# giltchcity/orb_slam3_ros

Measured on AMD Instinct MI355X. Metric: frames/sec ORB extract+match (752×480, 1000 kp) at 1/2/4/8 GPU; % HBM roofline, higher is better.
Workload: dtype u8; 1 GPU; EuRoC-MH01-like stereo 752x480 (BASELINE config 2): ORBextractor L+R (nFeatures=1000, scale 1.2, 8 levels, FAST 20/7) + ComputeStereoMatches; width=752, height=480, allgather=False, pipelines=1, parallelism=frame-sharded x1

## Files before the change

### include/orbfe.h

```cpp
#ifndef ORBFE_H
#define ORBFE_H

#include <stdint.h>

#ifdef __cplusplus
extern "C" {
#endif

#define ORBFE_OK 0
#define ORBFE_E_EMPTY (-1)
#define ORBFE_E_ARG (-2)
#define ORBFE_E_DEVICE (-3)
#define ORBFE_E_CAPACITY (-4)

typedef struct orbfe_keypoint {
    float x, y, size, angle, response;
    int32_t octave, class_id;
} orbfe_keypoint;

typedef struct orbfe_extractor orbfe_extractor;


int orbfe_extractor_create(int nfeatures, float scaleFactor, int nlevels, int iniThFAST, int minThFAST,
                           orbfe_extractor** out);
// ... 460 lines not shown
int orbfe_kfdb_detect_nbest(orbfe_kfdb* db, const uint32_t* q_word_ids, const double* q_weights, int32_t q_n,
                            const int32_t* connected_ids, int32_t n_connected, int32_t map_id,
                            const int32_t* bad_map_ids, int32_t n_bad_maps, int32_t n_candidates,
                            orbfe_kf_info_fn info, void* ctx, int32_t* loop_ids, int32_t* n_loop,
                            int32_t* merge_ids, int32_t* n_merge);

int orbfe_remap_linear_batch(const uint8_t* const* d_src, int sw, int sh, int sstride, const float* d_mapx,
                             const float* d_mapy, int dw, int dh, uint8_t* const* d_dst, int dstride, int n,
                             void* stream);
int orbfe_remap_linear(const uint8_t* src, int sw, int sh, int sstride, const float* mapx, const float* mapy, int dw,
                       int dh, uint8_t* dst, int dstride);

int orbfe_undistort_points(const float* pts, int n, const float* K4, const float* dist, int ndist, float* out);

int orbfe_matcher_set_timing(int enable);
float orbfe_matcher_last_ms(void);
int orbfe_matcher_set_stats(int enable);
int orbfe_matcher_last_stats(long long* out);
enum {
    ORBFE_SBP_FORM_NONE = 0,
    ORBFE_SBP_FORM_BLOCK = 1,
    ORBFE_SBP_FORM_MULTI = 2,
    ORBFE_SBP_FORM_BAND = 3,
    ORBFE_SBP_FORM_LOCAL = 4,
    ORBFE_SBP_FORM_LOCAL_WQ0 = 5,
    ORBFE_SBP_FORM_LOCAL_WQ1 = 6,
    ORBFE_SBP_FORM_LOCAL_WQ2 = 7,
    ORBFE_SBP_FORM_PROJ = 8,
    ORBFE_SBP_FORM_BLOCK4 = 9,
    ORBFE_SBP_FORM_BLOCK2 = 10,
    ORBFE_SBP_FORM_LOCAL2 = 11,
    ORBFE_SBP_FORM_PROJ2 = 12
};
int orbfe_matcher_last_form(void);
enum {
    ORBFE_BOW_FORM_NONE = 0,
    ORBFE_BOW_FORM_BLOCK = 1,
    ORBFE_BOW_FORM_NODES = 2,
    ORBFE_BOW_FORM_KFKF = 3
};
int orbfe_matcher_last_bow_form(void);
int orbfe_matcher_last_bow_batch(int32_t* out);
int orbfe_matcher_last_knn_form(int32_t* out);
int orbfe_matcher_last_bow_kf_batch(int32_t* out);
int orbfe_matcher_last_tri_batch(int32_t* out);
int orbfe_matcher_last_fuse_batch(int32_t* out);
int orbfe_matcher_last_track_batch(int32_t* out);
int orbfe_matcher_last_local_batch(int32_t* out);
int orbfe_matcher_last_local_uploads(void);
int orbfe_matcher_last_sim3_passes(void);

int orbfe_debug_copy(orbfe_extractor* h, int what, int image, int level, void* dst, int cap_bytes);

int orbfe_debug_fill_extractor(orbfe_extractor* h, uint32_t word, int64_t* bytes_out);

int orbfe_debug_fill_matcher(uint32_t word, int64_t bytes_out[3]);

int orbfe_debug_block_sort(uint64_t* data, int n);

const char* orbfe_version(void);

int orbfe_copy_stream(const void* d_src, void* d_dst, size_t bytes, void* stream);

#ifdef __cplusplus
}
#endif
#endif
```

### orb_slam3_ros_amd/_lib.py

```python
from __future__ import annotations

import ctypes
import os

_HERE = os.path.dirname(os.path.abspath(__file__))
LIB_PATH = os.path.join(_HERE, "liborbfe.so")
HEADER_PATH = os.path.join(os.path.dirname(_HERE), "include", "orbfe.h")

ORBFE_OK = 0
ORBFE_E_EMPTY = -1
ORBFE_E_ARG = -2
ORBFE_E_DEVICE = -3
ORBFE_E_CAPACITY = -4
ORBFE_NUM_STAGES = 3
STAGE_NAMES = ("pyramid_fast", "octree", "describe")


EPIPOLAR_FN = ctypes.CFUNCTYPE(ctypes.c_int32, ctypes.c_void_p, ctypes.c_int32, ctypes.c_int32)
KF_INFO_FN = ctypes.CFUNCTYPE(ctypes.c_int32, ctypes.c_void_p, ctypes.c_int32, ctypes.POINTER(ctypes.c_int32),
                              ctypes.POINTER(ctypes.c_int32))


class OrbKeyPoint(ctypes.Structure):
    _fields_ = [("x", ctypes.c_float), ("y", ctypes.c_float), ("size", ctypes.c_float),
                ("angle", ctypes.c_float), ("response", ctypes.c_float),
                ("octave", ctypes.c_int32), ("class_id", ctypes.c_int32)]


ORBFE_DEPTH_U16 = 0
ORBFE_DEPTH_F32 = 1


class RGBDParamsStruct(ctypes.Structure):
    _fields_ = [("fx", ctypes.c_float), ("fy", ctypes.c_float), ("cx", ctypes.c_float), ("cy", ctypes.c_float),
                ("dist", ctypes.c_float * 12), ("ndist", ctypes.c_int32), ("bf", ctypes.c_float),
                ("depth_factor", ctypes.c_float)]


class BowBatchStruct(ctypes.Structure):
    _fields_ = [("bow_word_ids", ctypes.c_void_p), ("bow_weights", ctypes.c_void_p), ("fv_node_ids", ctypes.c_void_p),
                ("fv_offsets", ctypes.c_void_p), ("fv_indices", ctypes.c_void_p), ("counts", ctypes.c_void_p)]


_c_int, _c_float, _vp = ctypes.c_int, ctypes.c_float, ctypes.c_void_p
_P_int, _P_float = ctypes.POINTER(ctypes.c_int), ctypes.POINTER(ctypes.c_float)

_SIGS = {
    "orbfe_extractor_create": (_c_int, [_c_int, _c_float, _c_int, _c_int, _c_int, ctypes.POINTER(_vp)]),
    "orbfe_extractor_destroy": (None, [_vp]),
    "orbfe_extractor_levels": (_c_int, [_vp]),
    "orbfe_extractor_scale_info": (_c_int, [_vp, _vp, _vp, _vp, _vp, _vp]),
    "orbfe_extractor_capacity": (_c_int, [_vp, _c_int, _c_int]),
    "orbfe_extract": (_c_int, [_vp, _vp, _c_int, _c_int, _c_int, _c_int, _c_int, _vp, _vp, _c_int, _P_int]),
    "orbfe_pyramid_level": (_c_int, [_vp, _c_int, _c_int, _vp, _c_int, _P_int, _P_int]),
    "orbfe_extract_batch": (_c_int, [_vp, _c_int, _vp, _c_int, _c_int, _c_int, _c_int, _c_int, _vp]),
    "orbfe_extract_batch_laps": (_c_int, [_vp, _c_int, _vp, _c_int, _c_int, _c_int, _vp, _vp]),
    "orbfe_batch_outputs": (_c_int, [_vp, ctypes.POINTER(_vp), ctypes.POINTER(_vp), ctypes.POINTER(_vp), _P_int]),
    "orbfe_set_stage_timing": (_c_int, [_vp, _c_int]),
    "orbfe_extractor_set_opencv_model": (_c_int, [_vp, _c_int, _c_int]),
    "orbfe_extractor_get_opencv_model": (_c_int, [_vp, _P_int, _P_int]),
    "orbfe_set_batch_outputs": (_c_int, [_vp, _vp, _vp, _vp, _c_int]),
    "orbfe_get_stage_timing": (_c_int, [_vp, _vp]),
    "orbfe_get_call_timing": (_c_int, [_vp, _vp]),
    "orbfe_stereo_match_batch": (_c_int, [_vp, _c_int, _c_int, _vp, _c_int, _c_int, _c_int, _c_float, _c_float,
                                          _vp, _vp, _vp, _vp]),
    "orbfe_stereo_match": (_c_int, [_vp, _vp, _c_float, _c_float, _vp, _vp]),
    "orbfe_frame_stereo": (_c_int, [_vp, _vp, _vp, _vp, _c_int, _c_int, _c_int, _c_float, _c_float,
                                    _vp, _vp, _c_int, _P_int, _P_int, _vp, _vp, _c_int, _P_int, _P_int, _vp, _vp]),
    "orbfe_frame_fisheye": (_c_int, [_vp, _vp, _vp, _vp, _c_int, _c_int, _c_int, _c_int, _c_int, _c_float,
                                     _vp, _vp, _c_int, _P_int, _P_int, _vp, _vp, _c_int, _P_int, _P_int, _vp, _vp]),
    "orbfe_descriptor_distance": (_c_int, [_vp, _vp]),
    "orbfe_debug_copy": (_c_int, [_vp, _c_int, _c_int, _c_int, _vp, _c_int]),
    "orbfe_debug_fill_extractor": (_c_int, [_vp, ctypes.c_uint32, ctypes.POINTER(ctypes.c_int64)]),
    "orbfe_debug_fill_matcher": (_c_int, [ctypes.c_uint32, ctypes.POINTER(ctypes.c_int64)]),
    "orbfe_debug_block_sort": (_c_int, [_vp, _c_int]),
    "orbfe_version": (ctypes.c_char_p, []),
    "orbfe_search_by_projection_local": (_c_int, [_vp, _vp, _vp, _vp, _c_int, _c_float, _c_int, _c_float, _c_float]),
    "orbfe_search_by_projection_lastframe": (_c_int, [_vp, _vp, _vp, _vp, _c_int, _c_float, _c_int, _c_int, _c_int]),
    "orbfe_search_by_projection_lastframe_stereo": (_c_int, [_vp, _vp, _vp, _vp, _vp, _c_int, _c_float, _c_int, _c_int,
                                                             _c_int]),
    "orbfe_search_by_projection_lastframe_pose": (_c_int, [_vp, _vp, _vp, _vp, _c_int, _vp, _vp, _vp, _c_float, _c_int,
                                                           _c_int, _c_int]),
    "orbfe_search_by_projection_kf": (_c_int, [_vp, _vp, _vp, _c_int, _c_float, _c_int, _c_int]),
    "orbfe_search_for_initialization": (_c_int, [_vp, _vp, _vp, _vp, _c_int, _c_float, _c_int]),
    "orbfe_search_by_bow": (_c_int, [_vp, _vp, _vp, _c_int, _vp, _vp, _vp, _vp, _c_float, _c_int]),
    "orbfe_copy_stream": (_c_int, [_vp, _vp, ctypes.c_size_t, _vp]),
    "orbfe_search_by_projection_local_device": (_c_int, [_vp, _vp, _vp, _vp, _c_int, _c_float, _c_int, _c_float,
                                                         _c_float, _vp]),
    "orbfe_search_local_points_device": (_c_int, [_vp, _vp, _vp, _c_int, _vp, _vp, _c_float, _c_int, _c_float,
                                                  _c_float, _vp, _vp]),
    "orbfe_search_by_bow_kf": (_c_int, [_vp, _vp, _vp, _c_int, _vp, _vp, _vp, _vp, _c_int, _vp, _vp, _c_float,
                                        _c_int]),
    "orbfe_distinctive_descriptors": (_c_int, [_vp, _vp, _c_int, _vp]),
    "orbfe_search_for_triangulation": (_c_int, [_vp, _vp, _vp, _vp, _vp, _vp, _vp, _vp, _vp, _c_int, _c_int, _c_int,
                                                _vp]),
    "orbfe_fuse": (_c_int, [_vp, _vp, _vp, _vp, _c_int, _c_float, _c_int, _vp, _vp]),
    "orbfe_search_by_projection_sim3": (_c_int, [_vp, _vp, _vp, _c_int, _vp, _c_int, _c_float, _vp, _vp]),
    "orbfe_search_by_projection_sim3_rig": (_c_int, [_vp, _vp, _vp, _vp, _c_int, _vp, _c_int, _c_float, _vp, _vp]),
    "orbfe_search_for_triangulation_epi": (_c_int, [_vp, _vp, _vp, _vp, _vp, _vp, _vp, _c_int, _c_int, EPIPOLAR_FN,
                                                    _vp, _vp]),
    "orbfe_search_by_sim3": (_c_int, [_vp, _vp, _vp, _vp, _vp, _vp, _vp, _vp, _c_float, _vp, _vp]),
    "orbfe_stereo_knn_ratio": (_c_int, [_vp, _c_int, _vp, _c_int, _c_float, _vp, _vp]),
    "orbfe_stereo_knn_slabs": (_c_int, [_vp, _vp, _c_int, _c_int, _vp, _vp, _c_int, _c_int, _c_int, _c_int, _c_float,
                                        _vp, _vp, _vp, _vp]),
    "orbfe_stereo_knn_batch": (_c_int, [_vp, _c_int, _c_int, _vp, _c_int, _c_int, _c_int, _c_float, _vp, _vp, _vp,
                                        _vp]),
    "orbfe_matcher_set_timing": (_c_int, [_c_int]),
    "orbfe_matcher_set_stats": (_c_int, [_c_int]),
    "orbfe_matcher_last_stats": (_c_int, [_vp]),
    "orbfe_matcher_last_form": (_c_int, []),
    "orbfe_matcher_last_bow_form": (_c_int, []),
    "orbfe_matcher_last_bow_batch": (_c_int, [_vp]),
    "orbfe_matcher_last_knn_form": (_c_int, [_vp]),
    "orbfe_matcher_last_sim3_passes": (_c_int, []),
    "orbfe_undistort_points": (_c_int, [_vp, _c_int, _vp, _vp, _c_int, _vp]),
    "orbfe_remap_linear": (_c_int, [_vp, _c_int, _c_int, _c_int, _vp, _vp, _c_int, _c_int, _vp, _c_int]),
    "orbfe_remap_linear_batch": (_c_int, [_vp, _c_int, _c_int, _c_int, _vp, _vp, _c_int, _c_int, _vp, _c_int, _c_int, _vp]),
    "orbfe_vocabulary_load_bin": (_c_int, [_vp, ctypes.c_size_t, ctypes.POINTER(_vp)]),
    "orbfe_vocabulary_create": (_c_int, [_c_int, _c_int, _c_int, _c_int, _c_int, _vp, _vp, _vp, _vp, ctypes.POINTER(_vp)]),
    "orbfe_vocabulary_destroy": (None, [_vp]),
    "orbfe_vocabulary_info": (_c_int, [_vp, _vp, _vp, _vp, _vp]),
    "orbfe_vocabulary_transform": (_c_int, [_vp, _vp, _c_int, _c_int, _vp, _vp, _vp, _vp, _vp, _vp, _vp]),
    "orbfe_is_in_frustum": (_c_int, [_vp, _vp, _vp, _c_int, _vp]),
    "orbfe_search_local_points": (_c_int, [_vp, _vp, _vp, _c_int, _vp, _vp, _c_float, _c_int, _c_float, _c_float, _vp]),
    "orbfe_matcher_last_ms": (_c_float, []),
    "orbfe_is_in_frustum_rig": (_c_int, [_vp, _vp, _vp, _vp, _c_int, _vp]),
# ... 101 lines not shown
```

### orb_slam3_ros_amd/csrc/orbfe_engine.hip

```cpp
#pragma clang fp contract(off)
#include <hip/hip_runtime.h>

#include <algorithm>
#include <atomic>
#include <cmath>
#include <cstdio>
#include <cstdlib>
#include <cstring>
#include <cstddef>
#include <mutex>
#include <vector>

#include "../../include/orbfe.h"
#include "orbfe_types.h"

#include "orbfe_kernels.hip"

using namespace orbfe;

#define HIPCHK(x)                                                                                 \
    do {                                                                                          \
        hipError_t e_ = (x);                                                                      \
        if (e_ != hipSuccess) {                                                                   \
            fprintf(stderr, "orbfe: HIP error %s at %s:%d\n", hipGetErrorString(e_), __FILE__, __LINE__); \
// ... 53 lines not shown
    double scale_factor;
    int resize_simd_lanes = 16;
    bool no_fused_pyramid = ab_knob("ORBFE_NO_FUSED_PYRAMID");
    bool fused_pyramid_batch = ab_knob("ORBFE_FUSED_PYR_BATCH");
    bool no_pull = ab_knob("ORBFE_NO_PULL");
    bool no_push = ab_knob("ORBFE_NO_PUSH");
    bool rgbd_mapped = ab_knob("ORBFE_RGBD_MAPPED");
    int blur_variant = 0;
    std::vector<float> scale, inv_scale, sigma2, inv_sigma2;
    std::vector<int> per_level;
    int device = 0;
    hipStream_t own_stream = nullptr;
    hipStream_t side_stream = nullptr;
    hipEvent_t ev_fork[ORBFE_MAX_LEVELS + 1] = {};
    int W = 0, H = 0, cap_b = 0;
    OrbGeom g{};
    std::vector<int16_t> tab;
    FastLds fast_lds{};
    FastLds fast_lds_lv[ORBFE_MAX_LEVELS] = {};
    size_t oct_lds = 0;
    std::vector<uint32_t> ptile;
    int pt_n = 0, pt_stride = 0, pt_cap = 0;
    size_t pt_lds = 0;
    int16_t* d_tab = nullptr;
    uint32_t* d_ptile = nullptr;
    uint8_t* d_pyr = nullptr;
    uint32_t* d_cellkeys = nullptr;
    int* d_cellcnt = nullptr;
    uint32_t* d_lkeys = nullptr;
    uint16_t* d_nodeof = nullptr;
    uint32_t* d_outkeys = nullptr;
    int* d_lvinfo = nullptr;
    int* d_ranks = nullptr;
    uint8_t* d_out = nullptr;
    OrbKeyPoint* d_kps = nullptr;
    uint8_t* d_desc = nullptr;
    int* d_counts = nullptr;
    const uint8_t** d_ptrs = nullptr;
    uint8_t* d_stage = nullptr;
    size_t stage_bytes = 0;
    uint8_t* h_pin = nullptr;
    size_t pin_bytes = 0;
    uint8_t* d_st = nullptr;
    float* d_uright = nullptr;
    float* d_depth = nullptr;
    int* d_nmatch = nullptr;
    int* d_sdist = nullptr;
    int sdist_frames = 0, sdist_kp = 0;
    int stereo_kp = 0;
    std::mutex mu_stereo;
    int last_nimg = 0, last_pitch = 0;
    int last_al0 = 0, last_builder[ORBFE_MAX_LEVELS] = {};
    int last_rs_rows[ORBFE_MAX_LEVELS] = {};
    uint64_t frame_id = 0, fs_id = 0;
    int fs_n = 0;
    float* d_scale = nullptr;
    uint8_t* d_rg = nullptr;
    float* d_rg_uright = nullptr;
    int rg_kp = 0;
    bool fs_rgbd = false;
    uint8_t* d_rg_stage = nullptr;
    size_t rg_stage_bytes = 0;
    const void** d_rg_ptrs = nullptr;
    int rg_ptrs_cap = 0;
    std::vector<const void*> last_rg_ptrs;
    std::vector<const uint8_t*> last_ptrs;
    std::vector<int> last_laps;
    bool timing = false;
    hipEvent_t ev[ORBFE_NUM_STAGES + 1] = {};
    hipEvent_t call_ev[7] = {};
    float call_ms[5] = {};
    std::vector<std::vector<hipEvent_t>> ev_ring;
    int ev_used = 0;
    float stage_ms[ORBFE_NUM_STAGES] = {};
    OrbKeyPoint* ext_kps = nullptr;
    uint8_t* ext_desc = nullptr;
    int* ext_counts = nullptr;
    int ext_cap_images = 0;
    OrbKeyPoint* last_kps = nullptr;
    uint8_t* last_desc = nullptr;
    int* last_counts = nullptr;
    std::mutex mu;
    unsigned long long* d_oct_ts = nullptr;
};

static void free_buffers(orbfe_extractor* h) {
    void** bufs[] = {(void**)&h->d_tab, (void**)&h->d_ptile, (void**)&h->d_pyr, (void**)&h->d_cellkeys,
                     (void**)&h->d_cellcnt, (void**)&h->d_lkeys, (void**)&h->d_nodeof, (void**)&h->d_outkeys,
                     (void**)&h->d_lvinfo, (void**)&h->d_ranks, (void**)&h->d_out, (void**)&h->d_ptrs};
    for (void** p : bufs) {
        if (*p) (void)hipFree(*p);
        *p = nullptr;
    }
    h->d_kps = nullptr;
    h->d_desc = nullptr;
    h->d_counts = nullptr;
    h->cap_b = 0;
    h->last_nimg = 0;
    h->last_kps = nullptr;
    h->last_desc = nullptr;
    h->last_counts = nullptr;
    h->last_ptrs.clear();
    h->last_laps.clear();
}

static int build_geom(const orbfe_extractor* h, int W, int H, OrbGeom& g, std::vector<int16_t>& tab,
// ... 359 lines not shown
    hipEvent_t* ev = nullptr;
    if (tm) {
        if (h->ev_used == (int)h->ev_ring.size()) {
            if (h->ev_ring.size() >= 1024) return ORBFE_E_CAPACITY;
            std::vector<hipEvent_t> set(ORBFE_NUM_STAGES + 1);
            for (auto& e : set) HIPCHK(hipEventCreate(&e));
            h->ev_ring.push_back(set);
        }
        ev = h->ev_ring[h->ev_used++].data();
        HIPCHK(hipEventRecord(ev[0], s));
    }
    const bool ext = use_ext && h->ext_kps;
    const bool small = B < kSmallBatch;
    OrbKeyPoint* o_kps = ext ? h->ext_kps : h->d_kps;
    uint8_t* o_desc = ext ? h->ext_desc : h->d_desc;
    int* o_counts = ext ? h->ext_counts : h->d_counts;
    {
        hipStream_t s2 = h->side_stream;
        auto fast_range = [&](hipStream_t st, int l0, int l1) {
            const int cpw = B < kSmallBatch ? 1 : l0 >= 4 ? 2 : 4;
            FastLds fl{0, 0, 0, 0};
            for (int l = l0; l < l1; l++) {
                fl.roi = std::max(fl.roi, h->fast_lds_lv[l].roi);
                fl.sc = std::max(fl.sc, h->fast_lds_lv[l].sc);
                fl.cor = std::max(fl.cor, h->fast_lds_lv[l].cor);
            }
            const int c0 = g.lv[l0].cell_base, c1 = l1 < g.nlevels ? g.lv[l1].cell_base : g.total_cells;
            fl.wave_bytes = fl.roi + fl.sc + fl.cor + FAST_ENT_BYTES;
            hipLaunchKernelGGL(k_fast, dim3((c1 - c0 + FAST_WPB * cpw - 1) / (FAST_WPB * cpw), B), dim3(64 * FAST_WPB),
                               (size_t)FAST_WPB * fl.wave_bytes, st, P, pitch, h->d_pyr, g.pyr_bytes, g, fl, h->d_cellkeys,
                               h->d_cellcnt, c0, c1, cpw);
        };
#ifdef FAST_NO_OVERLAP
        s2 = s;
#endif
        if (small) s2 = s;
        constexpr int kFastMid = 4;
        OrbGeom gr = g;
        if (B < kSmallBatch)
            for (int l = 1; l < g.nlevels; l++) gr.lv[l].rs_rows = std::min(g.lv[l].rs_rows, kSmallRsRows);
        const int lmid = std::min(std::max(kFastMid, 1), g.nlevels);
        const bool fork = s2 != s;
        if (fork) {
            HIPCHK(hipEventRecord(h->ev_fork[0], s));
            HIPCHK(hipStreamWaitEvent(s2, h->ev_fork[0], 0));
        }
        if (!small) fast_range(s2, 0, 1);
        bool al0 = (pitch & 3) == 0;
        for (int i = 0; al0 && i < B; i++) al0 = (((uintptr_t)host_ptrs[i]) & 3) == 0;
        const bool fused_pyr = h->pt_n > 0 && !h->no_fused_pyramid && (small || h->fused_pyramid_batch);
        h->last_al0 = al0 ? 1 : 0;
        for (int l = 1; l < g.nlevels; l++) h->last_builder[l] = fused_pyr ? 1 : (g.lv[l].rs_ok && (l > 1 || al0)) ? 2 : 3;
        for (int l = 1; l < g.nlevels; l++) h->last_rs_rows[l] = h->last_builder[l] == 2 ? gr.lv[l].rs_rows : 0;
        if (fused_pyr)
            hipLaunchKernelGGL(k_pyramid, dim3(h->pt_n, B), dim3(PYR_NT), h->pt_lds, s, P, pitch, h->d_pyr, g.pyr_bytes, g,
                               h->d_ptile, h->pt_stride, h->pt_cap, al0 ? 1 : 0);
        for (int l = 1; l < g.nlevels && !fused_pyr; l++) {
            const OrbLevel& L = g.lv[l];
            if (L.rs_ok && (l > 1 || al0)) {
                const int rows = gr.lv[l].rs_rows;
                const int nstrips = (L.w + RS_COLS - 1) / RS_COLS, nitems = nstrips * ((L.h + rows - 1) / rows);
                hipLaunchKernelGGL(k_resize_s, dim3((nitems + RS_WPB - 1) / RS_WPB, B), dim3(64 * RS_WPB), 0, s, P, pitch, h->d_pyr,
                                   g.pyr_bytes, h->d_tab, gr, l, nstrips, nitems);
            } else {
                const int tiles_y = (L.h + L.rz_rows - 1) / L.rz_rows;
                dim3 grid((L.w + L.rz_cols - 1) / L.rz_cols, (tiles_y + RZ_TPB - 1) / RZ_TPB, B);
                hipLaunchKernelGGL(k_resize, grid, dim3(256), 0, s, P, pitch, h->d_pyr, g.pyr_bytes, h->d_tab, g, l);
            }
            if (l + 1 == lmid && !small) {
                if (fork) {
                    HIPCHK(hipEventRecord(h->ev_fork[2], s));
                    HIPCHK(hipStreamWaitEvent(s2, h->ev_fork[2], 0));
                }
                fast_range(s2, 1, lmid);
            }
        }
        if (small) {
            fast_range(s, 0, g.nlevels);
        } else {
            if (fork) HIPCHK(hipEventRecord(h->ev_fork[1], s2));
            if (fused_pyr) fast_range(s, 1, g.nlevels);
            else if (lmid < g.nlevels) fast_range(s, lmid, g.nlevels);
            if (fork) HIPCHK(hipStreamWaitEvent(s, h->ev_fork[1], 0));
        }
    }
    BlurKernel bk;
    memcpy(bk.k, h->blur_variant == 1 ? kBlurRound : kBlurED, sizeof(bk.k));
    if (tm) HIPCHK(hipEventRecord(ev[1], s));
    if (small) {
        hipLaunchKernelGGL(k_octree<kSmallOctNt>, dim3(B, g.nlevels), dim3(kSmallOctNt), h->oct_lds, s, g,
                           h->d_cellkeys, h->d_cellcnt, h->d_lkeys, h->d_nodeof, h->d_outkeys, h->d_lvinfo,
                           h->d_ranks, d_laps, h->d_oct_ts, 0);
    } else {
        hipLaunchKernelGGL(k_octree<OCT_NT>, dim3(B, g.nlevels), dim3(OCT_NT), h->oct_lds, s, g, h->d_cellkeys, h->d_cellcnt,
                           h->d_lkeys, h->d_nodeof, h->d_outkeys, h->d_lvinfo, h->d_ranks, d_laps, h->d_oct_ts, 0);
    }
    if (tm) HIPCHK(hipEventRecord(ev[2], s));
    if (B < kSmallBatch)
        hipLaunchKernelGGL(k_describe<1>, dim3((g.out_per_img + DP_WPB - 1) / DP_WPB, B), dim3(64 * DP_WPB), 0, s, P,
                           pitch, h->d_pyr, g.pyr_bytes, g, h->d_outkeys, h->d_lvinfo, h->d_ranks, o_kps, o_desc,
                           o_counts, bk);
    else
        hipLaunchKernelGGL(k_describe<DP_KPW>, dim3((g.out_per_img + DP_WPB * DP_KPW - 1) / (DP_WPB * DP_KPW), B),
                           dim3(64 * DP_WPB), 0, s, P, pitch, h->d_pyr, g.pyr_bytes, g, h->d_outkeys, h->d_lvinfo,
                           h->d_ranks, o_kps, o_desc, o_counts, bk);
    if (tm) HIPCHK(hipEventRecord(ev[3], s));
    HIPCHK(hipGetLastError());
    h->last_kps = o_kps;
    h->last_desc = o_desc;
    h->last_counts = o_counts;
    return ORBFE_OK;
}

static hipStream_t pick_stream(orbfe_extractor* h, void* stream) {
    (void)h;
    return (hipStream_t)stream;
// ... 616 lines not shown
    if (frame_id == 0 || left->fs_id != frame_id || left->frame_id != frame_id || !left->last_kps ||
        !(left->fs_rgbd ? (void*)left->d_rg : (void*)left->d_st))
        return ORBFE_E_ARG;
    if (!left->d_scale) {
        HIPCHK(hipSetDevice(left->device));
        HIPCHK(hipMalloc(&left->d_scale, ORBFE_MAX_LEVELS * sizeof(float)));
        HIPCHK(hipMemcpy(left->d_scale, left->scale.data(), left->nlevels * sizeof(float), hipMemcpyHostToDevice));
    }
    F->n = left->fs_n;
    F->keys = (const orbfe_keypoint*)left->last_kps;
    F->desc = left->last_desc;
    F->uright = left->d_uright;
    if (left->fs_rgbd) {
        F->keys = (const orbfe_keypoint*)left->d_rg;
        F->uright = left->d_rg_uright;
    }
    F->nlevels = left->nlevels;
    F->scale_factors = left->d_scale;
    F->two_cams = 0;
    F->nleft = 0;
    F->l2r = F->r2l = nullptr;
    F->device = 1;
    return ORBFE_OK;
}

int orbfe_debug_copy(orbfe_extractor* h, int what, int image, int level, void* dst, int cap_bytes) {
    if (!h || !h->cap_b || image < 0 || image >= h->last_nimg || level < 0 || level >= h->nlevels) return ORBFE_E_ARG;
    HIPCHK(hipDeviceSynchronize());
    const OrbGeom& g = h->g;
    const OrbLevel& L = g.lv[level];
    const int ncell = L.n_cols * L.n_rows;
    const void* src = nullptr;
    size_t bytes = 0;
    int count = 0;
    int info[4];
    HIPCHK(hipMemcpy(info, h->d_lvinfo + ((size_t)image * g.nlevels + level) * 4, 16, hipMemcpyDeviceToHost));
    if (what == 0) { src = h->d_cellcnt + (size_t)image * g.total_cells + L.cell_base; count = ncell; bytes = 4 * count; }
    else if (what == 1) { src = h->d_cellkeys + (size_t)image * g.cellkeys_per_img + L.cellkey_off; count = ncell * L.cell_cap; bytes = 4 * (size_t)count; }
    else if (what == 2) { src = h->d_outkeys + (size_t)image * g.out_per_img + L.out_off; count = info[0]; bytes = 4 * (size_t)count; }
    else if (what == 3) { if (cap_bytes < 16) return ORBFE_E_CAPACITY; memcpy(dst, info, 16); return 4; }
    else if (what == 5) {
        if (cap_bytes < 16) return ORBFE_E_CAPACITY;
        const int path[4] = {h->pt_n, level ? h->last_builder[level] : 0, L.rs_ok, h->last_al0};
        memcpy(dst, path, 16);
        return 4;
    }
    else if (what == 6) {
        if (cap_bytes < 24) return ORBFE_E_CAPACITY;
        const int geo[6] = {level ? L.rz_rows : 0, level ? L.rz_cols : 0, level ? h->last_rs_rows[level] : 0,
                            level ? L.simd_end : 0, level ? L.xmax : 0, level ? L.pitch : h->last_pitch};
        memcpy(dst, geo, 24);
        return 6;
    }
    else if (what == 4) {
        if (!h->d_oct_ts) return 0;
        src = h->d_oct_ts + 64 * level; count = 64; bytes = 64 * 8;
    }
    else return ORBFE_E_ARG;
    if (!dst) return count;
    if ((size_t)cap_bytes < bytes) return ORBFE_E_CAPACITY;
    if (bytes) HIPCHK(hipMemcpy(dst, src, bytes, hipMemcpyDeviceToHost));
    return count;
}

int orbfe_debug_fill_extractor(orbfe_extractor* h, uint32_t word, int64_t* bytes_out) {
    if (bytes_out) *bytes_out = 0;
    if (!h) return ORBFE_E_ARG;
    std::lock_guard<std::mutex> lk(h->mu);
    std::lock_guard<std::mutex> lks(h->mu_stereo);
    const OrbGeom& g = h->g;
    const size_t B = (size_t)h->cap_b;
    size_t o_kps = 0, o_desc = 0, o_end = 0;
    if (h->cap_b) out_layout(h->cap_b, g.kp_cap, &o_kps, &o_desc, &o_end);
    auto a16 = [](size_t b) { return (b + 15) & ~(size_t)15; };
    const struct { void* p; size_t bytes; } dev[] = {
        {h->d_pyr, B * g.pyr_bytes},
        {h->d_cellkeys, B * g.cellkeys_per_img * 4},
        {h->d_cellcnt, B * g.total_cells * 4},
        {h->d_lkeys, B * g.cellkeys_per_img * 4},
        {h->d_nodeof, B * g.cellkeys_per_img * 2},
        {h->d_outkeys, B * g.out_per_img * 4},
        {h->d_lvinfo, B * g.nlevels * 4 * 4},
        {h->d_ranks, B * g.out_per_img * 4},
        {h->d_out, o_end},
        {h->d_stage, h->stage_bytes},
        {h->d_st, 16 + (size_t)h->stereo_kp * 8},
        {h->d_sdist, (size_t)h->sdist_frames * h->sdist_kp * 4},
        {h->d_rg, a16(a16((size_t)h->rg_kp * sizeof(OrbKeyPoint)) + (size_t)h->rg_kp * 8)},
        {h->d_rg_stage, h->rg_stage_bytes},
    };
    int64_t total = 0;
    bool any = h->h_pin != nullptr;
    for (const auto& b : dev) any = any || (b.p && b.bytes >= 4);
    if (!any) return ORBFE_OK;
    HIPCHK(hipSetDevice(h->device));
    HIPCHK(hipDeviceSynchronize());
    hipStream_t s = h->own_stream;
    for (const auto& b : dev) {
        if (!b.p || b.bytes < 4) continue;
        HIPCHK(hipMemsetD32Async((hipDeviceptr_t)b.p, (int)word, b.bytes / 4, s));
        total += (int64_t)(b.bytes / 4 * 4);
    }
    HIPCHK(hipStreamSynchronize(s));
    if (h->h_pin) {
        std::fill_n((uint32_t*)h->h_pin, h->pin_bytes / 4, word);
        total += (int64_t)(h->pin_bytes / 4 * 4);
    }
    if (bytes_out) *bytes_out = total;
    return ORBFE_OK;
}

#if ORBFE_OCT_STAMPS
int orbfe_debug_sort_stamps(uint64_t* out) {
    HIPCHK(hipMemcpyFromSymbol(out, HIP_SYMBOL(g_sort_ts), (16 * 16 + 16) * 8));
    return 272;
// ... 70 lines not shown
```

### orb_slam3_ros_amd/csrc/orbfe_kernels.hip

```cpp
#pragma clang fp contract(off)
#include <hip/hip_runtime.h>
#include <float.h>
#include <math.h>
#include <stdint.h>

#include <type_traits>

#include "brief_pattern.h"
#include "glibc_sincosf.h"
#include "orbfe_types.h"
#include "stl_sort.h"

namespace orbfe {

#define SYNC() __syncthreads()
#define WAVE_SYNC()                                               \
    do {                                                          \
        __builtin_amdgcn_fence(__ATOMIC_RELEASE, "workgroup");    \
        __builtin_amdgcn_s_waitcnt(0xc07f);                       \
        __builtin_amdgcn_wave_barrier();                          \
        __builtin_amdgcn_fence(__ATOMIC_ACQUIRE, "workgroup");    \
    } while (0)

__constant__ int c_umax[16] = {15, 15, 15, 15, 14, 14, 14, 13, 13, 12, 11, 10, 9, 8, 6, 3};
// ... 225 lines not shown
            nsr = ty[4 * (y1 - 1) + 1] - sr0 + 1;
            fetch(y0, y1, sr0, nsr);
        }
        if (hr0 < hstep) {
            const uint32_t a0 = (hlin ? (uint32_t)ha0 : 2048u) << 4, a1 = (hlin ? (uint32_t)ha1 : 0u) << 4;
            for (int r = hr0; r < cnsr; r += hstep) {
                const uint32_t p0 = s_src[r][hsx], p1 = s_src[r][hsx + 1];
                s_h[r][hx] = (int)((__umul24(p0, a0) + __umul24(p1, a1)) & hmask);
            }
        }
        SYNC();
        if (vact) {
            for (int dy = cy0 + rl; dy < cy1; dy += rstep) {
                const int* tyr = s_ty[dy - cy0];
                const int r0 = tyr[0] - csr0, r1 = tyr[1] - csr0;
                const uint32_t b0s = (uint32_t)tyr[2], b1s = (uint32_t)tyr[3];
                const int4 H0 = *(const int4*)&s_h[r0][4 * cg];
                const int4 H1 = *(const int4*)&s_h[r1][4 * cg];
                const uint32_t h0[4] = {(uint32_t)H0.x, (uint32_t)H0.y, (uint32_t)H0.z, (uint32_t)H0.w};
                const uint32_t h1[4] = {(uint32_t)H1.x, (uint32_t)H1.y, (uint32_t)H1.z, (uint32_t)H1.w};
                uint32_t packed = 0;
                if (all_vec) {
#pragma unroll
                    for (int q = 0; q < 4; q++) {
                        const uint32_t vv = (mulhi_u24(h0[q], b0s) + mulhi_u24(h1[q], b1s) + 2) >> 2;
                        packed |= vv << (8 * q);
                    }
                } else {
                    const uint32_t b0 = b0s >> 8, b1 = b1s >> 8;
#pragma unroll
                    for (int q = 0; q < 4; q++) {
                        const uint32_t vs = (mulhi_u24(h0[q], b0s) + mulhi_u24(h1[q], b1s) + 2) >> 2;
                        const uint32_t vl = (__umul24(h0[q] >> 4, b0) + __umul24(h1[q] >> 4, b1) + (1u << 21)) >> 22;
                        packed |= (vec[q] ? vs : vl) << (8 * q);
                    }
                }
                uint8_t* dp = dst + (size_t)dy * L.pitch + xq;
                if (xq + 4 <= x1) {
                    *(uint32_t*)dp = packed;
                } else {
                    for (int q = 0; q < 4 && xq + q < x1; q++) dp[q] = (uint8_t)(packed >> (8 * q));
                }
            }
        }
        SYNC();
    }
}

#define RS_D 5
#define RS_ROWS 48
#define RS_COLS 256
typedef unsigned short orbfe_ushort2_rs __attribute__((ext_vector_type(2)));
#define RS_WPB 4
__device__ __forceinline__ void resize_s_item(const uint8_t* const* imgs, int in_pitch, uint8_t* pyr, int pyr_stride,
                                              const int16_t* __restrict__ tab, const OrbGeom& g, int l, int nstrips,
                                              int item, int b) {
    const OrbLevel& L = g.lv[l];
    const int lane = lane_id();
    const int chunk = item / nstrips, strip = item - chunk * nstrips;
    const int y0 = chunk * L.rs_rows, y1 = min(y0 + L.rs_rows, L.h);
    int spitch;
    gptr_u8 src = level_base(imgs, in_pitch, pyr, pyr_stride, g, b, l - 1, &spitch);
    uint8_t* dst = pyr + (size_t)b * pyr_stride + L.pyr_off;
    const int16_t* tx = tab + L.tab_x;
    const int16_t* ty = tab + L.tab_y;
    const int xq = strip * RS_COLS + 4 * lane;
    const bool act = xq < L.w;
    const int base = tx[3 * min(xq, L.w - 1)] & ~3;
    uint32_t sel[4], coef[4], hmask[4];
    bool vec[4];
#pragma unroll
    for (int q = 0; q < 4; q++) {
        const int x = min(xq + q, L.w - 1);
        const bool lin = x < L.xmax;
        const uint32_t a0 = lin ? (uint32_t)tx[3 * x + 1] : 2048u, a1 = lin ? (uint32_t)tx[3 * x + 2] : 0u;
        const uint32_t off = (uint32_t)(tx[3 * x] - base) - (q >= 2 ? 2u : 0u);
        sel[q] = 0x0c000c00u | (off & 7u) | (((off + 1u) & 7u) << 16);
        coef[q] = (a0 << 4) | (a1 << 20);
        vec[q] = x < L.simd_end;
        hmask[q] = vec[q] ? 0xFFFF00u : 0xFFFFFFFFu;
    }
    const bool lv_all = !act || (vec[0] && vec[1] && vec[2] && vec[3]);
    int t_s0 = 0, t_r1 = 0, t_b0 = 0, t_b1 = 0;
    if (y0 + lane < y1) {
        const int16_t* tr = ty + 4 * (y0 + lane);
        t_s0 = tr[0];
        t_r1 = tr[1];
        t_b0 = (int)tr[2] << 8;
        t_b1 = (int)tr[3] << 8;
    }
    const int s_lo = __builtin_amdgcn_readfirstlane(t_s0);
    const int s_hi = ty[4 * (y1 - 1) + 1];
    int y = y0;
    int r1 = __builtin_amdgcn_readfirstlane(t_r1);
    uint32_t b0s = (uint32_t)__builtin_amdgcn_readfirstlane(t_b0), b1s = (uint32_t)__builtin_amdgcn_readfirstlane(t_b1);
    uint8_t* drow = dst + (size_t)y0 * L.pitch + xq;
    uint32_t* slack = (uint32_t*)(pyr + (size_t)b * pyr_stride + g.pyr_slack) + lane;
    uint32_t Hp[4] = {0u, 0u, 0u, 0u};
    auto step = [&](int s, uint32_t w0, uint32_t w1, uint32_t w2) {
        const uint32_t c0 = __builtin_amdgcn_alignbyte(w1, w0, 2u), c1 = __builtin_amdgcn_alignbyte(w2, w1, 2u);
        uint32_t Hc[4];
#pragma unroll
        for (int q = 0; q < 4; q++) {
            const uint32_t pr = q < 2 ? __builtin_amdgcn_perm(w1, w0, sel[q]) : __builtin_amdgcn_perm(c1, c0, sel[q]);
            Hc[q] = __builtin_amdgcn_udot2(__builtin_bit_cast(orbfe_ushort2_rs, pr),
                                           __builtin_bit_cast(orbfe_ushort2_rs, coef[q]), 0u, false) &
                    hmask[q];
        }
        const bool fin = r1 == s;
        uint32_t packed = 0;
        if (fin) {
#pragma unroll
            for (int q = 0; q < 4; q++)
                packed |= ((mulhi_u24(Hp[q], b0s) + mulhi_u24(Hc[q], b1s) + 2u) >> 2) << (8 * q);
            if (!lv_all) {
                const uint64_t b0 = b0s >> 8, b1 = b1s >> 8;
#pragma unroll
                for (int q = 0; q < 4; q++) {
                    const uint32_t vl = (uint32_t)(((uint64_t)Hp[q] * b0 + (uint64_t)Hc[q] * b1 + (1ull << 25)) >> 26);
                    const uint32_t m = vec[q] ? 0u : 0xFFu << (8 * q);
                    packed = (packed & ~m) | ((vl << (8 * q)) & m);
                }
            }
        }
        *(uint32_t*)(fin && act ? (uint32_t*)drow : slack) = packed;
        if (fin) {
            drow += L.pitch;
            if (++y == y1) {
                r1 = -1;
            } else {
                const int k = y - y0;
                r1 = __builtin_amdgcn_readlane(t_r1, k);
                b0s = (uint32_t)__builtin_amdgcn_readlane(t_b0, k);
                b1s = (uint32_t)__builtin_amdgcn_readlane(t_b1, k);
            }
        }
#pragma unroll
        for (int q = 0; q < 4; q++) Hp[q] = Hc[q];
    };
    const uint32_t win = (uint32_t)min(base, spitch - 4);
    const uint64_t sp = (uint64_t)(uintptr_t)src;
    const uint32_t sp_lo = __builtin_amdgcn_readfirstlane((uint32_t)sp), sp_hi = __builtin_amdgcn_readfirstlane((uint32_t)(sp >> 32));
    const int sbytes = __builtin_amdgcn_readfirstlane(spitch * g.lv[l - 1].h);
    const __amdgpu_buffer_rsrc_t srd =
        __builtin_amdgcn_make_buffer_rsrc((void*)(((uint64_t)sp_hi << 32) | sp_lo), (short)0, sbytes, 0x00020000);
    auto ld = [&](int s, uint32_t (&w)[3]) {
        const int so = __builtin_amdgcn_readfirstlane(s * spitch);
        typedef uint32_t u32x3 __attribute__((ext_vector_type(3)));
        const u32x3 v = __builtin_bit_cast(u32x3, __builtin_amdgcn_raw_buffer_load_b96(srd, (int)win, so, 0));
        w[0] = v.x; w[1] = v.y; w[2] = v.z;
    };
    uint32_t buf[RS_D][3];
#pragma unroll
    for (int d = 0; d < RS_D; d++) {
        *slack = 0u;
        ld(min(s_lo + d, s_hi), buf[d]);
        __builtin_amdgcn_sched_barrier(0);
    }
    for (int sb = s_lo; sb <= s_hi; sb += RS_D) {
#pragma unroll
        for (int d = 0; d < RS_D; d++) {
            step(sb + d, buf[d][0], buf[d][1], buf[d][2]);
            ld(min(sb + RS_D + d, s_hi), buf[d]);
            __builtin_amdgcn_sched_barrier(0);
        }
    }
}
__global__ __launch_bounds__(64 * RS_WPB) void k_resize_s(const uint8_t* const* imgs, int in_pitch, uint8_t* pyr,
                                                  int pyr_stride, const int16_t* __restrict__ tab, OrbGeom g, int l,
                                                  int nstrips, int nitems) {
    const int wave = __builtin_amdgcn_readfirstlane(threadIdx.x >> 6);
    const int lb = xcd_logical(block_linear(), gridDim.x * gridDim.y);
    const int bx = lb % gridDim.x, b = lb / gridDim.x;
    const int item = bx * RS_WPB + wave;
    if (item >= nitems) return;
    resize_s_item(imgs, in_pitch, pyr, pyr_stride, tab, g, l, nstrips, item, b);
}

#ifndef PYR_NT
#define PYR_NT 1024
#endif
#define PYR_RU 2
#ifndef PYR_U0
#define PYR_U0 4
#endif
__global__ __launch_bounds__(PYR_NT) void k_pyramid(const uint8_t* const* imgs, int in_pitch, uint8_t* pyr, int pyr_stride,
                                                    OrbGeom g, const uint32_t* __restrict__ ptile, int pt_stride, int cap,
                                                    int al0) {
    extern __shared__ __attribute__((aligned(16))) uint8_t smem_pyr[];
    const int lb = xcd_logical(block_linear(), gridDim.x * gridDim.y);
    const int tile = lb % gridDim.x, b = lb / gridDim.x;
    const int tid = threadIdx.x;
    uint32_t* srec = (uint32_t*)smem_pyr;
    uint8_t* buf0 = smem_pyr + (size_t)pt_stride * 4;
    uint8_t* buf1 = buf0 + cap;
    const uint32_t* rec = ptile + (size_t)tile * pt_stride;
    const uint32_t hx = rec[0], hy = rec[1];
    const int ax0 = (int)(hx & 0xffff), ax1 = (int)(hx >> 16), ny0 = (int)(hy & 0xffff), ny1 = (int)(hy >> 16);
    const int dpr = (ax1 - ax0) >> 2, items0 = dpr * (ny1 - ny0);
    const int W0 = g.lv[0].w;
    gptr_u8 src = as_global(imgs[b]);
    orbfe_u32x4 rv[PYR_RU];
#pragma unroll
    for (int u = 0; u < PYR_RU; u++) {
        const int i = tid + PYR_NT * u;
        if (i < (pt_stride >> 2)) rv[u] = ((const ORBFE_GLOBAL orbfe_u32x4*)rec)[i];
    }
    uint32_t wv[PYR_U0];
#pragma unroll
    for (int u = 0; u < PYR_U0; u++) {
        const int i = tid + PYR_NT * u;
        wv[u] = 0u;
        if (i < items0) {
            const int r = small_div(i, dpr), c = i - r * dpr;
            const int x = ax0 + 4 * c;
            gptr_u8 sp = src + (size_t)(ny0 + r) * in_pitch + x;
            if (al0 && x + 4 <= W0) {
                wv[u] = *(const ORBFE_GLOBAL uint32_t*)sp;
            } else {
                uint32_t w = 0u;
                for (int k = 0; k < 4; k++)
                    if (x + k < W0) w |= (uint32_t)sp[k] << (8 * k);
                wv[u] = w;
            }
        }
    }
#pragma unroll
    for (int u = 0; u < PYR_RU; u++) {
        const int i = tid + PYR_NT * u;
// ... 2100 lines not shown
```

Before: 162,300 frames/s.

## Pack partial-width resize tail strips into shared waves across row chunks

In the per-level resize kernel, the last partial column strip used to take one wave per row chunk while leaving most lanes idle. It is now handled by a packed path where each wave splits its lanes into groups, each group working on a different row chunk. That path stages the row interpolation table in LDS and streams source rows through a buffer resource. It only runs on the chained (non-fused) pyramid path, and a debug entry point is added to force that path. The cost is extra LDS use and added kernel complexity.

Measured after the change: 165,000 frames/s, median of 6. +1.7%, better.

```diff
diff --git a/include/orbfe.h b/include/orbfe.h
--- a/include/orbfe.h
+++ b/include/orbfe.h
@@ -536,6 +536,8 @@
 
 int orbfe_debug_copy(orbfe_extractor* h, int what, int image, int level, void* dst, int cap_bytes);
 
+int orbfe_debug_chained_pyramid(orbfe_extractor* h, int on);
+
 int orbfe_debug_fill_extractor(orbfe_extractor* h, uint32_t word, int64_t* bytes_out);
 
 int orbfe_debug_fill_matcher(uint32_t word, int64_t bytes_out[3]);
diff --git a/orb_slam3_ros_amd/_lib.py b/orb_slam3_ros_amd/_lib.py
--- a/orb_slam3_ros_amd/_lib.py
+++ b/orb_slam3_ros_amd/_lib.py
@@ -72,6 +72,7 @@
     "orbfe_descriptor_distance": (_c_int, [_vp, _vp]),
     "orbfe_debug_copy": (_c_int, [_vp, _c_int, _c_int, _c_int, _vp, _c_int]),
     "orbfe_debug_fill_extractor": (_c_int, [_vp, ctypes.c_uint32, ctypes.POINTER(ctypes.c_int64)]),
+    "orbfe_debug_chained_pyramid": (_c_int, [_vp, _c_int]),
     "orbfe_debug_fill_matcher": (_c_int, [ctypes.c_uint32, ctypes.POINTER(ctypes.c_int64)]),
     "orbfe_debug_block_sort": (_c_int, [_vp, _c_int]),
     "orbfe_version": (ctypes.c_char_p, []),
diff --git a/orb_slam3_ros_amd/csrc/orbfe_engine.hip b/orb_slam3_ros_amd/csrc/orbfe_engine.hip
--- a/orb_slam3_ros_amd/csrc/orbfe_engine.hip
+++ b/orb_slam3_ros_amd/csrc/orbfe_engine.hip
@@ -129,6 +129,7 @@
     int last_nimg = 0, last_pitch = 0;
     int last_al0 = 0, last_builder[ORBFE_MAX_LEVELS] = {};
     int last_rs_rows[ORBFE_MAX_LEVELS] = {};
+    int last_rs_pack[ORBFE_MAX_LEVELS][4] = {};
     uint64_t frame_id = 0, fs_id = 0;
     int fs_n = 0;
     float* d_scale = nullptr;
@@ -594,16 +595,27 @@
         h->last_al0 = al0 ? 1 : 0;
         for (int l = 1; l < g.nlevels; l++) h->last_builder[l] = fused_pyr ? 1 : (g.lv[l].rs_ok && (l > 1 || al0)) ? 2 : 3;
         for (int l = 1; l < g.nlevels; l++) h->last_rs_rows[l] = h->last_builder[l] == 2 ? gr.lv[l].rs_rows : 0;
+        memset(h->last_rs_pack, 0, sizeof h->last_rs_pack);
         if (fused_pyr)
             hipLaunchKernelGGL(k_pyramid, dim3(h->pt_n, B), dim3(PYR_NT), h->pt_lds, s, P, pitch, h->d_pyr, g.pyr_bytes, g,
                                h->d_ptile, h->pt_stride, h->pt_cap, al0 ? 1 : 0);
         for (int l = 1; l < g.nlevels && !fused_pyr; l++) {
             const OrbLevel& L = g.lv[l];
             if (L.rs_ok && (l > 1 || al0)) {
-                const int rows = gr.lv[l].rs_rows;
-                const int nstrips = (L.w + RS_COLS - 1) / RS_COLS, nitems = nstrips * ((L.h + rows - 1) / rows);
-                hipLaunchKernelGGL(k_resize_s, dim3((nitems + RS_WPB - 1) / RS_WPB, B), dim3(64 * RS_WPB), 0, s, P, pitch, h->d_pyr,
-                                   g.pyr_bytes, h->d_tab, gr, l, nstrips, nitems);
+                const int rows = gr.lv[l].rs_rows, nchunks = (L.h + rows - 1) / rows;
+                int nstrips = (L.w + RS_COLS - 1) / RS_COLS;
+                const int r = small ? 0 : rs_pack_lanes(L.w), G = rs_pack_groups(r, rows);
+                int npacked = 0;
+                if (G >= 2) {
+                    nstrips--;
+                    npacked = (nchunks + G - 1) / G;
+                }
+                const int nfull = nstrips * nchunks, nitems = nfull + npacked;
+                const int pack[4] = {npacked ? r : 0, npacked ? G : 0, nfull, npacked};
+                memcpy(h->last_rs_pack[l], pack, sizeof pack);
+                const size_t lds = npacked ? (size_t)RS_WPB * rs_pack_entries(r, rows, L.h) * sizeof(uint2) : 0;
+                hipLaunchKernelGGL(k_resize_s, dim3((nitems + RS_WPB - 1) / RS_WPB, B), dim3(64 * RS_WPB), lds, s, P, pitch, h->d_pyr,
+                                   g.pyr_bytes, h->d_tab, gr, l, nstrips, nitems, nfull, npacked ? r : 0);
             } else {
                 const int tiles_y = (L.h + L.rz_rows - 1) / L.rz_rows;
                 dim3 grid((L.w + L.rz_cols - 1) / L.rz_cols, (tiles_y + RZ_TPB - 1) / RZ_TPB, B);
@@ -1326,6 +1338,11 @@
         memcpy(dst, geo, 24);
         return 6;
     }
+    else if (what == 7) {
+        if (cap_bytes < 16) return ORBFE_E_CAPACITY;
+        memcpy(dst, h->last_rs_pack[level], 16);
+        return 4;
+    }
     else if (what == 4) {
         if (!h->d_oct_ts) return 0;
         src = h->d_oct_ts + 64 * level; count = 64; bytes = 64 * 8;
@@ -1335,6 +1352,13 @@
     if ((size_t)cap_bytes < bytes) return ORBFE_E_CAPACITY;
     if (bytes) HIPCHK(hipMemcpy(dst, src, bytes, hipMemcpyDeviceToHost));
     return count;
+}
+
+int orbfe_debug_chained_pyramid(orbfe_extractor* h, int on) {
+    if (!h) return ORBFE_E_ARG;
+    std::lock_guard<std::mutex> lk(h->mu);
+    h->no_fused_pyramid = on != 0;
+    return ORBFE_OK;
 }
 
 int orbfe_debug_fill_extractor(orbfe_extractor* h, uint32_t word, int64_t* bytes_out) {
diff --git a/orb_slam3_ros_amd/csrc/orbfe_kernels.hip b/orb_slam3_ros_amd/csrc/orbfe_kernels.hip
--- a/orb_slam3_ros_amd/csrc/orbfe_kernels.hip
+++ b/orb_slam3_ros_amd/csrc/orbfe_kernels.hip
@@ -301,6 +301,65 @@
 #define RS_COLS 256
 typedef unsigned short orbfe_ushort2_rs __attribute__((ext_vector_type(2)));
 #define RS_WPB 4
+#define RS_PK_ROWS 512
+__host__ __device__ inline int rs_pack_lanes(int w) { return ((w % RS_COLS) + 3) >> 2; }
+__host__ __device__ inline int rs_pack_groups(int r, int rows) {
+    const int a = r ? 64 / r : 0, b = RS_PK_ROWS / rows;
+    return a < b ? a : b;
+}
+__host__ __device__ inline int rs_pack_entries(int r, int rows, int h) {
+    const int n = rs_pack_groups(r, rows) * rows;
+    return (n < h ? n : h) + 1;
+}
+struct RsCols {
+    uint32_t sel[4], coef[4], hmask[4];
+    bool vec[4];
+};
+__device__ __forceinline__ int rs_columns(const int16_t* tx, const OrbLevel& L, int xq, RsCols& C) {
+    const int base = tx[3 * min(xq, L.w - 1)] & ~3;
+#pragma unroll
+    for (int q = 0; q < 4; q++) {
+        const int x = min(xq + q, L.w - 1);
+        const bool lin = x < L.xmax;
+        const uint32_t a0 = lin ? (uint32_t)tx[3 * x + 1] : 2048u, a1 = lin ? (uint32_t)tx[3 * x + 2] : 0u;
+        const uint32_t off = (uint32_t)(tx[3 * x] - base) - (q >= 2 ? 2u : 0u);
+        C.sel[q] = 0x0c000c00u | (off & 7u) | (((off + 1u) & 7u) << 16);
+        C.coef[q] = (a0 << 4) | (a1 << 20);
+        C.vec[q] = x < L.simd_end;
+        C.hmask[q] = C.vec[q] ? 0xFFFF00u : 0xFFFFFFFFu;
+    }
+    return base;
+}
+template <bool LATE>
+__device__ __forceinline__ void rs_hsums(const RsCols& C, uint32_t w0, uint32_t w1, uint32_t w2, uint32_t (&Hc)[4]) {
+    const uint32_t c0 = __builtin_amdgcn_alignbyte(w1, w0, 2u), c1 = __builtin_amdgcn_alignbyte(w2, w1, 2u);
+#pragma unroll
+    for (int q = 0; q < 4; q++) {
+        const uint32_t pr = q < 2 ? __builtin_amdgcn_perm(w1, w0, C.sel[q]) : __builtin_amdgcn_perm(c1, c0, C.sel[q]);
+        Hc[q] = __builtin_amdgcn_udot2(__builtin_bit_cast(orbfe_ushort2_rs, pr),
+                                       __builtin_bit_cast(orbfe_ushort2_rs, C.coef[q]), 0u, false) &
+                (LATE ? 0xFFFFFFFFu : C.hmask[q]);
+    }
+}
+template <bool LATE>
+__device__ __forceinline__ uint32_t rs_vertical(const RsCols& C, const uint32_t (&Hp)[4], const uint32_t (&Hc)[4],
+                                                uint32_t b0s, uint32_t b1s, bool tail) {
+    const uint32_t m = LATE ? 0xFFFF00u : 0xFFFFFFFFu;
+    uint32_t packed = 0;
+#pragma unroll
+    for (int q = 0; q < 4; q++)
+        packed |= ((mulhi_u24(Hp[q] & m, b0s) + mulhi_u24(Hc[q] & m, b1s) + 2u) >> 2) << (8 * q);
+    if (tail) {
+        const uint64_t b0 = b0s >> 8, b1 = b1s >> 8;
+#pragma unroll
+        for (int q = 0; q < 4; q++) {
+            const uint32_t vl = (uint32_t)(((uint64_t)Hp[q] * b0 + (uint64_t)Hc[q] * b1 + (1ull << 25)) >> 26);
+            const uint32_t m = C.vec[q] ? 0u : 0xFFu << (8 * q);
+            packed = (packed & ~m) | ((vl << (8 * q)) & m);
+        }
+    }
+    return packed;
+}
 __device__ __forceinline__ void resize_s_item(const uint8_t* const* imgs, int in_pitch, uint8_t* pyr, int pyr_stride,
                                               const int16_t* __restrict__ tab, const OrbGeom& g, int l, int nstrips,
                                               int item, int b) {
@@ -315,21 +374,9 @@
     const int16_t* ty = tab + L.tab_y;
     const int xq = strip * RS_COLS + 4 * lane;
     const bool act = xq < L.w;
-    const int base = tx[3 * min(xq, L.w - 1)] & ~3;
-    uint32_t sel[4], coef[4], hmask[4];
-    bool vec[4];
-#pragma unroll
-    for (int q = 0; q < 4; q++) {
-        const int x = min(xq + q, L.w - 1);
-        const bool lin = x < L.xmax;
-        const uint32_t a0 = lin ? (uint32_t)tx[3 * x + 1] : 2048u, a1 = lin ? (uint32_t)tx[3 * x + 2] : 0u;
-        const uint32_t off = (uint32_t)(tx[3 * x] - base) - (q >= 2 ? 2u : 0u);
-        sel[q] = 0x0c000c00u | (off & 7u) | (((off + 1u) & 7u) << 16);
-        coef[q] = (a0 << 4) | (a1 << 20);
-        vec[q] = x < L.simd_end;
-        hmask[q] = vec[q] ? 0xFFFF00u : 0xFFFFFFFFu;
-    }
-    const bool lv_all = !act || (vec[0] && vec[1] && vec[2] && vec[3]);
+    RsCols C;
+    const int base = rs_columns(tx, L, xq, C);
+    const bool lv_all = !act || (C.vec[0] && C.vec[1] && C.vec[2] && C.vec[3]);
     int t_s0 = 0, t_r1 = 0, t_b0 = 0, t_b1 = 0;
     if (y0 + lane < y1) {
         const int16_t* tr = ty + 4 * (y0 + lane);
@@ -347,31 +394,11 @@
     uint32_t* slack = (uint32_t*)(pyr + (size_t)b * pyr_stride + g.pyr_slack) + lane;
     uint32_t Hp[4] = {0u, 0u, 0u, 0u};
     auto step = [&](int s, uint32_t w0, uint32_t w1, uint32_t w2) {
-        const uint32_t c0 = __builtin_amdgcn_alignbyte(w1, w0, 2u), c1 = __builtin_amdgcn_alignbyte(w2, w1, 2u);
         uint32_t Hc[4];
-#pragma unroll
-        for (int q = 0; q < 4; q++) {
-            const uint32_t pr = q < 2 ? __builtin_amdgcn_perm(w1, w0, sel[q]) : __builtin_amdgcn_perm(c1, c0, sel[q]);
-            Hc[q] = __builtin_amdgcn_udot2(__builtin_bit_cast(orbfe_ushort2_rs, pr),
-                                           __builtin_bit_cast(orbfe_ushort2_rs, coef[q]), 0u, false) &
-                    hmask[q];
-        }
+        rs_hsums<false>(C, w0, w1, w2, Hc);
         const bool fin = r1 == s;
         uint32_t packed = 0;
-        if (fin) {
-#pragma unroll
-            for (int q = 0; q < 4; q++)
-                packed |= ((mulhi_u24(Hp[q], b0s) + mulhi_u24(Hc[q], b1s) + 2u) >> 2) << (8 * q);
-            if (!lv_all) {
-                const uint64_t b0 = b0s >> 8, b1 = b1s >> 8;
-#pragma unroll
-                for (int q = 0; q < 4; q++) {
-                    const uint32_t vl = (uint32_t)(((uint64_t)Hp[q] * b0 + (uint64_t)Hc[q] * b1 + (1ull << 25)) >> 26);
-                    const uint32_t m = vec[q] ? 0u : 0xFFu << (8 * q);
-                    packed = (packed & ~m) | ((vl << (8 * q)) & m);
-                }
-            }
-        }
+        if (fin) packed = rs_vertical<false>(C, Hp, Hc, b0s, b1s, !lv_all);
         *(uint32_t*)(fin && act ? (uint32_t*)drow : slack) = packed;
         if (fin) {
             drow += L.pitch;
@@ -415,15 +442,102 @@
         }
     }
 }
+__device__ __forceinline__ void resize_s_item_packed(const uint8_t* const* imgs, int in_pitch, uint8_t* pyr, int pyr_stride,
+                                                     const int16_t* __restrict__ tab, const OrbGeom& g, int l, int nstrips,
+                                                     int item, int b, int r, uint2* s_tab) {
+    const OrbLevel& L = g.lv[l];
+    const int lane = lane_id();
+    const int rows = L.rs_rows, G = rs_pack_groups(r, rows);
+    const int grp = small_div(lane, r), lg = lane - grp * r;
+    const int16_t* ty = tab + L.tab_y;
+    const int R0 = item * G * rows, nrw = min(G * rows, L.h - R0);
+    for (int i = lane; i <= nrw; i += 64) {
+        const int16_t* tr = ty + 4 * (R0 + min(i, nrw - 1));
+        const int c0 = small_div(i, rows) * rows;
+        const int rel = i == c0 || i == nrw ? -1 : tr[1] - ty[4 * (R0 + c0)];
+        s_tab[i] = make_uint2((uint32_t)rel, (uint32_t)(uint16_t)tr[2] | ((uint32_t)(uint16_t)tr[3] << 16));
+    }
+    WAVE_SYNC();
+    const bool live = grp < G && R0 + grp * rows < L.h;
+    const int y0 = live ? R0 + grp * rows : R0, ylast = min(y0 + rows, L.h) - 1;
+    int ti = y0 - R0;
+    const uint2 e0 = s_tab[ti];
+    const int s_lo = ty[4 * y0], s_hi = ty[4 * ylast + 1];
+    int span = live ? s_hi - s_lo + 1 : 0;
+#pragma unroll
+    for (int d = 32; d >= 1; d >>= 1) span = max(span, __shfl_xor(span, d, 64));
+    const int nsteps = __builtin_amdgcn_readfirstlane(span);
+    int spitch;
+    gptr_u8 src = level_base(imgs, in_pitch, pyr, pyr_stride, g, b, l - 1, &spitch);
+    uint8_t* img = pyr + (size_t)b * pyr_stride;
+    const int xq = nstrips * RS_COLS + 4 * lg;
+    RsCols C;
+    const int base = rs_columns(tab + L.tab_x, L, xq, C);
+    const bool lv_all = !live || (C.vec[0] && C.vec[1] && C.vec[2] && C.vec[3]);
+    const bool tail = __builtin_amdgcn_ballot_w64(!lv_all) != 0;
+    int r1 = live ? ty[4 * y0 + 1] - s_lo : -1;
+    uint32_t b0s = (e0.y & 0xFFFFu) << 8, b1s = (e0.y >> 16) << 8;
+    uint2 nxt = s_tab[++ti];
+    uint32_t doff = (uint32_t)L.pyr_off + (uint32_t)y0 * (uint32_t)L.pitch + (uint32_t)xq;
+    const uint32_t soff = (uint32_t)g.pyr_slack + 4u * (uint32_t)lane;
+    uint32_t Hp[4] = {0u, 0u, 0u, 0u};
+    auto step = [&](int k, uint32_t w0, uint32_t w1, uint32_t w2) {
+        uint32_t Hc[4];
+        rs_hsums<true>(C, w0, w1, w2, Hc);
+        const bool fin = r1 == k;
+        const uint32_t packed = rs_vertical<true>(C, Hp, Hc, b0s, b1s, tail);
+        *(uint32_t*)(img + (fin ? doff : soff)) = packed;
+        doff += fin ? (uint32_t)L.pitch : 0u;
+        r1 = fin ? (int)nxt.x : r1;
+        b0s = fin ? (nxt.y & 0xFFFFu) << 8 : b0s;
+        b1s = fin ? (nxt.y >> 16) << 8 : b1s;
+        ti = min(ti + (fin ? 1 : 0), nrw);
+        nxt = s_tab[ti];
+#pragma unroll
+        for (int q = 0; q < 4; q++) Hp[q] = Hc[q];
+    };
+    const uint64_t sp = (uint64_t)(uintptr_t)src;
+    const uint32_t sp_lo = __builtin_amdgcn_readfirstlane((uint32_t)sp), sp_hi = __builtin_amdgcn_readfirstlane((uint32_t)(sp >> 32));
+    const int sbytes = __builtin_amdgcn_readfirstlane(spitch * g.lv[l - 1].h);
+    const __amdgpu_buffer_rsrc_t srd =
+        __builtin_amdgcn_make_buffer_rsrc((void*)(((uint64_t)sp_hi << 32) | sp_lo), (short)0, sbytes, 0x00020000);
+    const int win = min(base, spitch - 4);
+    int lo = win + s_lo * spitch;
+    const int lo_hi = win + s_hi * spitch;
+    auto ld = [&](uint32_t (&w)[3]) {
+        typedef uint32_t u32x3 __attribute__((ext_vector_type(3)));
+        const u32x3 v = __builtin_bit_cast(u32x3, __builtin_amdgcn_raw_buffer_load_b96(srd, lo, 0, 0));
+        w[0] = v.x; w[1] = v.y; w[2] = v.z;
+        lo = min(lo + spitch, lo_hi);
+    };
+    uint32_t buf[RS_D][3];
+#pragma unroll
+    for (int d = 0; d < RS_D; d++) {
+        *(uint32_t*)(img + soff) = 0u;
+        ld(buf[d]);
+        __builtin_amdgcn_sched_barrier(0);
+    }
+    for (int kb = 0; kb < nsteps; kb += RS_D) {
+#pragma unroll
+        for (int d = 0; d < RS_D; d++) {
+            step(kb + d, buf[d][0], buf[d][1], buf[d][2]);
+            ld(buf[d]);
+            __builtin_amdgcn_sched_barrier(0);
+        }
+    }
+}
 __global__ __launch_bounds__(64 * RS_WPB) void k_resize_s(const uint8_t* const* imgs, int in_pitch, uint8_t* pyr,
                                                   int pyr_stride, const int16_t* __restrict__ tab, OrbGeom g, int l,
-                                                  int nstrips, int nitems) {
+                                                  int nstrips, int nitems, int nfull, int pk_r) {
+    extern __shared__ uint2 s_tab[];
     const int wave = __builtin_amdgcn_readfirstlane(threadIdx.x >> 6);
     const int lb = xcd_logical(block_linear(), gridDim.x * gridDim.y);
     const int bx = lb % gridDim.x, b = lb / gridDim.x;
     const int item = bx * RS_WPB + wave;
     if (item >= nitems) return;
-    resize_s_item(imgs, in_pitch, pyr, pyr_stride, tab, g, l, nstrips, item, b);
+    if (item < nfull) resize_s_item(imgs, in_pitch, pyr, pyr_stride, tab, g, l, nstrips, item, b);
+    else resize_s_item_packed(imgs, in_pitch, pyr, pyr_stride, tab, g, l, nstrips, item - nfull, b, pk_r,
+                              s_tab + wave * rs_pack_entries(pk_r, g.lv[l].rs_rows, g.lv[l].h));
 }
 
 #ifndef PYR_NT
```
